# iacopo97/Multimodal-SAM-Adapter

Hardware: AMD Instinct MI355X
Metric: images/sec encoder fwd @1024x1024 RGB+LiDAR ViT-L (higher is better)
Workload: dtype split-operand MFMA: fp16 hi + e5m2 cross terms (h8c / h8 planes, ViT / interaction / up-conv GEMMs) fp16 hi/lo pairs x3 (TwinConvNeXt: f3 planes) and bf16 hi/lo x3 (neck, head); attention blocks with the rel-pos terms fused: every contraction on one fp16 MFMA (q, k, v, P rounded to fp16) in the bloc

## Files before the change

include/mmsa.h:

```cpp
#ifndef MMSA_H
#define MMSA_H
#include <stddef.h>
#include <stdint.h>
#ifdef __cplusplus
extern "C" {
#endif

#ifdef MMSA_BUILDING_LIBRARY
typedef hipStream_t mmsa_stream_t;
#else
typedef void* mmsa_stream_t;
#endif

#include "mmsa_version.h"
int mmsa_version(void);
const char* mmsa_last_error(void);

int mmsa_debug_poison_lds(unsigned pattern, mmsa_stream_t stream);
int mmsa_event_create(void** ev);
int mmsa_event_record(void* ev, mmsa_stream_t stream);
int mmsa_event_elapsed_ms(void* start, void* stop, float* ms);
int mmsa_event_destroy(void* ev);

enum { MMSA_ACT_NONE = 0, MMSA_ACT_GELU = 1, MMSA_ACT_RELU = 2, MMSA_ACT_RELU6 = 3, MMSA_ACT_HSWISH = 4, MMSA_ACT_SIGMOID = 5 };

enum { MMSA_DT_F32 = 0, MMSA_DT_F16 = 1, MMSA_DT_F64 = 2 };

enum { MMSA_FMT_B3 = 0, MMSA_FMT_H8 = 1, MMSA_FMT_H8C = 2, MMSA_FMT_F3 = 3, MMSA_FMT_W8 = 4  };

int mmsa_ms_deform_attn_forward(const void* value, const int64_t* spatial_shapes, const int64_t* level_start_index,
                                const void* sampling_loc, const void* attn_weight, void* out, int batch,
                                int spatial_size, int num_heads, int channels, int num_levels, int num_query,
                                int num_point, int im2col_step, int dtype, mmsa_stream_t stream);

int mmsa_ms_deform_attn_backward(const void* value, const int64_t* spatial_shapes, const int64_t* level_start_index,
                                 const void* sampling_loc, const void* attn_weight, const void* grad_output,
                                 void* grad_value, void* grad_sampling_loc, void* grad_attn_weight, int batch,
                                 int spatial_size, int num_heads, int channels, int num_levels, int num_query,
                                 int num_point, int im2col_step, int dtype, mmsa_stream_t stream);

int mmsa_msda_fused(const float* value, const int64_t* spatial_shapes, const int64_t* level_start_index,
                    const float* raw, long ldraw, const float* ref_points, float* out, long ldo,
                    uint16_t* out_planes, long ldop , int out_fmt , int batch,
                    int spatial_size, int num_heads, int channels, int num_levels, int num_query, int num_point,
                    float* clamp_max , mmsa_stream_t stream);

int mmsa_msda_fused_planes(const uint16_t* value_planes, long ldvp, int lo_bytes, const int64_t* spatial_shapes, const int64_t* level_start_index,
                           const float* raw, long ldraw, const float* ref_points, float* out, long ldo,
                           uint16_t* out_planes, long ldop, int out_fmt, int batch,
                           int spatial_size, int num_heads, int channels, int num_levels, int num_query, int num_point,
                           float* clamp_max, mmsa_stream_t stream);

int mmsa_rowstats_finalize(const float* rowstats, int rows, int strips, int D, float eps, float* mean_rstd, mmsa_stream_t stream);

int mmsa_zero_bytes(void* p, size_t bytes, mmsa_stream_t stream);
int mmsa_gemm_split3(const float* A, const uint16_t* Ap, long lda, long strideA,
                     const uint16_t* Wp, long strideW,
                     const float* bias, long strideBias, const float* colscale, const float* resid, long ldr,
                     long strideR, int resid_mod, float beta, float* C, long ldc, long strideC,
                     uint16_t* Cp, long ldcp, long strideCp, int M, int N, int K,
                     int batch, int act, float alpha, int out_mode, int ps_H, int ps_W, int ps_C, int fmt, int cp_fmt,
                     int max_grid, float* rowstats_out, const float* rownorm_mean_rstd, const float* rownorm_colsum, int flavour,
                     float* clamp_max , mmsa_stream_t stream);

int mmsa_convnext_mlp_fused(const uint16_t* Ap, long lda, long strideA, const uint16_t* W1p, long strideW1, const uint16_t* W2p,
                            long strideW2, const float* b1, const float* b2, const float* gamma, float* x, long ldx, long strideX,
                            int M, int C, int batch, int max_grid, int fmt,
                            float* clamp_max , mmsa_stream_t stream);

int mmsa_split_planes(const float* src, long ld, int rows, int cols, int cols_pad, uint16_t* planes, int kind,
                      float* clamp_max , mmsa_stream_t stream);

int mmsa_attention(const float* qkv, long ldq, const float* qkv_bias, const float* rp, float* out, long ldo, int B,
                   int H, int W, int heads, int head_dim, int window_size, float scale, mmsa_stream_t stream);
int mmsa_attention_planes(const uint16_t* qkv_planes, long ldq, const uint16_t* bias_planes, const float* rp,
                          uint16_t* out_planes, long ldo, int B, int H, int W, int heads, int head_dim,
                          int window_size, float scale, int out_fmt ,
                          int v_fmt ,
                          float* max_abs_logit , mmsa_stream_t stream);

int mmsa_relpos_bias(const float* qkv, long ldq, const float* Rh, const float* Rw, float* rp, int B, int H, int W,
                     int heads, int head_dim, int window_size, mmsa_stream_t stream);
int mmsa_relpos_bias_planes(const uint16_t* qkv_planes, long ldq, const float* Rh, const float* Rw,
                            float* rp, int B, int H, int W, int heads, int head_dim, int window_size, mmsa_stream_t stream);

int mmsa_layernorm_rows(const float* x, long ldx, const float* w, const float* b, float eps, float* y, long ldy,
                        float* y2, long ldy2, uint16_t* y_planes, long ldp ,
                        int rows, int C, int map_mode, int map_H, int map_W, int group_rows, long w_gstride, long y_gcol,
                        int y_wrap, int plane_fmt , float* clamp_max ,
                        mmsa_stream_t stream);

int mmsa_colstats(const float* x, long ldx, long strideB, const float* wrow, int B, int HW, int C, double* out,
                  int out_is_zero , mmsa_stream_t stream);

int mmsa_ffrm_finalize(const double* stats, int B, int HW, int C, float mean_w, float mean_b, const float* Wc,
                       const float* gn_w, const float* gn_b, float* mean_o, float* rstd_o, float* mult_o,
                       float* scratch , mmsa_stream_t stream);
int mmsa_lnhw_apply(const float* x, long ldx, const float* mean, const float* rstd, const float* mult, const float* w,
                    const float* bias, float* y, long ldy, int B, int HW, int C, mmsa_stream_t stream);

int mmsa_dwconv_nhwc(const float* x, long ldx, long xstrideB, const float* w, const float* bias, float* y, long ldy,
                     long ystrideB, uint16_t* y_planes, long ldp, long pstrideB , int planes_fmt ,
                     int B, int H, int W, int C, int k, int act,
                     int imgs_per_group ,
                     float* rowstats ,
                     float* clamp_max , mmsa_stream_t stream);
int mmsa_gconv_nhwc(const float* x, long ldx, const float* w, const float* bias, float* y, long ldy, int B, int H,
                    int W, int G, int cin_g, int cout_g, int k, int act, mmsa_stream_t stream);
int mmsa_gfe_qkv_conv(const float* x, long ldx, const float* w, float* y, long ldy, int B, int H, int W, int G, int cin_g, int cout_g,
                      int* covered, mmsa_stream_t stream);
int mmsa_dwpair_gate(const float* x, long ldx, const float* w, float* y, long ldy, uint16_t* y_planes, long ldp, int B, int H,
                     int W, int C, mmsa_stream_t stream);
int mmsa_im2col_nchw(const float* x, int B, int Ctot, int c0, int Cin, int H, int W, int p, float* out, int Kpad,
                     mmsa_stream_t stream);

long mmsa_gram_tn_scratch_bytes(int B, int P, int c);
int mmsa_gram_tn(const float* X, long ldx, const float* Y, long ldy, long strideB, double* G , int B, int P, int c,
                 int nblk, void* scratch, long scratch_bytes, mmsa_stream_t stream);
int mmsa_chanattn_build(const double* G, const double* sq, long sq_strideB, const double* sk, long sk_strideB,
                        const float* temp, const float* Wp, uint16_t* planes , int B, int c, int cpad,
                        int heads, mmsa_stream_t stream);
int mmsa_gffm_build(const double* E, uint16_t* x_planes, uint16_t* y_planes , int B, int c,
                    int cpad, mmsa_stream_t stream);
int mmsa_gelu_gate(const float* x, long ldx, float* y, long ldy, long rows, int C, mmsa_stream_t stream);
int mmsa_pool_hw(const float* z, long ldz, float* out, long ldo, int B, int H, int W, int C, mmsa_stream_t stream);
int mmsa_ca_apply(const float* z, long ldz, const float* att, long lda, float* out, long ldo,
                  uint16_t* out_planes, long ldp , int B, int H, int W, int C, mmsa_stream_t stream);

int mmsa_tail_fuse(const float* cmap, long ldc, long cstrideB, const float* xtok, long ldx, const float* bn_scale,
                   const float* bn_shift, float* out, uint16_t* out_planes , long ldp,
                   int B, int Hc, int Wc, int Hx, int Wx, int C, mmsa_stream_t stream);

int mmsa_global_attention_planes(const uint16_t* qkv_planes, long ldq, const uint16_t* bias_planes, const uint16_t* relpos_planes,
                                 uint16_t* out_planes, long ldo, int B, int H, int W, int heads, int head_dim, float scale,
                                 int out_fmt , int v_fmt ,
                                 float* max_abs_logit , mmsa_stream_t stream);

int mmsa_window_attention_planes(const uint16_t* qkv_planes, long ldq, const uint16_t* bias_planes,
                                 const uint16_t* relpos_planes, const uint16_t* selector, uint16_t* out_planes, long ldo, int B, int H, int W,
                                 int heads, int head_dim, int window_size, float scale, int out_fmt ,
                                 int v_fmt , float* max_abs_logit , mmsa_stream_t stream);

int mmsa_nchw_to_planes(const float* src, long strideB, uint16_t* planes, long ldp, int B, int C, long HW,
                        mmsa_stream_t stream);
int mmsa_head_fuse(const float* z0, const float* z1, int H1, int W1, const float* z2, int H2, int W2, const float* z3,
                   int H3, int W3, long ld, const float* bn_scale, const float* bn_shift, uint16_t* planes, long ldp,
                   float* out32, long ldo, int B, int H, int W, int C, int act, mmsa_stream_t stream);
int mmsa_tokens_to_nchw(const float* src, long ld, float* dst, int B, long HW, int C, mmsa_stream_t stream);

int mmsa_bilinear_accum_nchw(const float* src, long src_strideB, int B, int C, int hs, int ws, float* dst, int Hd, int Wd, int y0, int x0,
                             int hc, int wc, float* count, int accumulate, mmsa_stream_t stream);
int mmsa_div_count_nchw(float* x, const float* count, int B, int C, long HW, mmsa_stream_t stream);
int mmsa_argmax_nchw(const float* x, unsigned char* out, int B, int C, long HW, mmsa_stream_t stream);
int mmsa_crop_batch_nchw(const float* src, int B, int C, int H, int W, const int* windows, int n, float* dst, int hc, int wc,
                         mmsa_stream_t stream);
int mmsa_slide_argmax(const float* logits, int n, int C, int hs, int ws, const int* windows, unsigned char* out, int B, int H, int W,
                      int hc, int wc, int* uncovered, mmsa_stream_t stream);
int mmsa_slide_argmax_resized(const float* logits, int n, int C, int hs, int ws, const int* windows, unsigned char* out, int B, int H, int W,
                              int hc, int wc, int Hd, int Wd, int Hcut, int Wcut, int* uncovered, mmsa_stream_t stream);

enum { MMSA_PRE_U8 = 0, MMSA_PRE_F32 = 1 };
int mmsa_preprocess_nhwc(const void* src0, int dtype0, const void* src1, int dtype1, int B, int Hs, int Ws, const float* mean,
                         const float* sinv, const int* div255, const int* swap, const float* pad_val, float* dst, int H, int W,
                         mmsa_stream_t stream);
int mmsa_preprocess_crops(const void* src0, int dtype0, const void* src1, int dtype1, int B, int Hs, int Ws, const float* mean,
                          const float* sinv, const int* div255, const int* swap, const float* pad_val, int H, int W, const int* windows,
                          int n, float* dst, int hc, int wc, mmsa_stream_t stream);
int mmsa_preprocess_resize_nhwc(const void* src0, int dtype0, const void* src1, int dtype1, int B, int Hs, int Ws, const float* mean,
                                const float* sinv, const int* div255, const int* swap, const float* pad_val, float* dst, int H, int W,
                                int Hr, int Wr, const int* xofs, const void* xcoef, const int* yofs, const void* ycoef, int fixed_point,
                                mmsa_stream_t stream);
int mmsa_preprocess_resize_crops(const void* src0, int dtype0, const void* src1, int dtype1, int B, int Hs, int Ws, const float* mean,
                                 const float* sinv, const int* div255, const int* swap, const float* pad_val, int H, int W, const int* windows,
                                 int n, float* dst, int hc, int wc, int Hr, int Wr, const int* xofs, const void* xcoef, const int* yofs,
                                 const void* ycoef, int fixed_point, mmsa_stream_t stream);

int mmsa_eval_confusion_u8(const unsigned char* pred, const unsigned char* label, int B, int H, int W, int Hl, int Wl, const unsigned char* lut,
                           int C, const int* ymap, const int* xmap, const int* slots, int n_slots, int64_t* counts, mmsa_stream_t stream);
int mmsa_slide_argmax_eval(const float* logits, int n, int C, int hs, int ws, const int* windows, unsigned char* out, int B, int H, int W,
                           int hc, int wc, int* uncovered, const unsigned char* label, int Hl, int Wl, const unsigned char* lut, const int* ymap,
                           const int* xmap, const int* slots, int n_slots, int64_t* counts, mmsa_stream_t stream);

int mmsa_render_u8(const unsigned char* pred, long pred_image_stride, long pred_row_stride, int B, int h, int w, const unsigned* palette, int npal,
                   int palette_reverse, const unsigned char* src, int Hs, int Ws, int src_reverse, double opacity, double one_minus_opacity,
                   unsigned char* out, mmsa_stream_t stream);
int mmsa_render_denorm_f32(const unsigned char* pred, long pred_image_stride, long pred_row_stride, int B, int h, int w, const unsigned* palette, int npal,
                           int palette_reverse, const float* src, int Cs, int Hs, int Ws, const float* mean, const float* std, int to_rgb, int mul255,
                           double opacity, double one_minus_opacity, unsigned char* out, mmsa_stream_t stream);

#ifdef __cplusplus
}
#endif
#endif
```

include/mmsa_version.h:

```cpp
#ifndef MMSA_VERSION_H
#define MMSA_VERSION_H
#define MMSA_ABI_VERSION 109
#endif
```

multimodal-sam-adapter_amd/mmsa/head.py:

```python
import torch
import torch.nn as nn

from . import lib
from . import ops
from .params import Node, _attach


class SegformerHead(nn.Module):
    def __init__(self, interpolate_mode="bilinear", in_channels=None, channels=None, *, num_classes=None, dropout_ratio=0.1,
                 conv_cfg=None, norm_cfg=None, act_cfg=dict(type="ReLU"), in_index=-1, input_transform="multiple_select",
                 loss_decode=None, ignore_index=255, sampler=None, align_corners=False, init_cfg=None, **kwargs):
        super().__init__()
        if in_channels is None or channels is None or num_classes is None:
            raise TypeError("SegformerHead: in_channels, channels and num_classes are required")
        if not isinstance(in_channels, (list, tuple)) or not isinstance(in_index, (list, tuple)) or len(in_channels) != len(in_index):
            raise AssertionError("SegformerHead: in_channels and in_index must be lists of equal length")
        if not 1 <= len(in_channels) <= 4:
            raise NotImplementedError("mmsa SegformerHead: 1..4 input maps")
        if interpolate_mode != "bilinear" or align_corners:
            raise NotImplementedError("mmsa SegformerHead: only interpolate_mode='bilinear', align_corners=False (the reference configs)")
        if norm_cfg is None or norm_cfg.get("type") not in ("BN", "SyncBN"):
            raise NotImplementedError("mmsa SegformerHead: norm_cfg must be BN / SyncBN (eval: running-statistics affine)")
        if act_cfg is None or act_cfg.get("type") != "ReLU":
            raise NotImplementedError("mmsa SegformerHead: act_cfg must be ReLU")
        if channels % 8:
            raise NotImplementedError("mmsa SegformerHead: channels must be a multiple of 8")
        self.in_channels, self.in_index, self.channels = list(in_channels), list(in_index), channels
        self.num_classes, self.dropout_ratio, self.align_corners = num_classes, dropout_ratio, align_corners
        self.interpolate_mode, self.ignore_index, self.norm_cfg, self.act_cfg = interpolate_mode, ignore_index, norm_cfg, act_cfg
        n = len(in_channels)
        g = torch.Generator().manual_seed(0)

        def conv_w(co, ci):
            return torch.randn(co, ci, 1, 1, generator=g) * (2.0 / ci) ** 0.5

        def bn(prefix):
            _attach(self, prefix + ".weight", torch.ones(channels))
            _attach(self, prefix + ".bias", torch.zeros(channels))
            _attach(self, prefix + ".running_mean", torch.zeros(channels), buffer=True)
            _attach(self, prefix + ".running_var", torch.ones(channels), buffer=True)
            _attach(self, prefix + ".num_batches_tracked", torch.zeros((), dtype=torch.long), buffer=True)

        _attach(self, "conv_seg.weight", torch.randn(num_classes, channels, 1, 1, generator=g) * 0.01)
        _attach(self, "conv_seg.bias", torch.zeros(num_classes))
        self.add_module("convs", Node())
        for i, ci in enumerate(in_channels):
            _attach(self, f"convs.{i}.conv.weight", conv_w(channels, ci))
            bn(f"convs.{i}.bn")
        _attach(self, "fusion_conv.conv.weight", conv_w(channels, channels * n))
        bn("fusion_conv.bn")
        self._packed = None
        self._bufs = {}
        self.register_load_state_dict_post_hook(lambda m, _: m.invalidate())
        self.eval()

    def invalidate(self):
        self._packed = None

    def train(self, mode=True):
        if mode:
            raise NotImplementedError("mmsa: the MI355X decode head implements the inference forward path only")
        return super().train(False)

    def init_weights(self):
        pass

    def forward_test(self, inputs, img_metas=None, test_cfg=None):
        return self.forward(inputs)

    def forward_train(self, inputs, img_metas, gt_semantic_seg, train_cfg):
        raise NotImplementedError("mmsa: the MI355X decode head implements the inference forward path only (no losses)")

    @torch.no_grad()
    def _pack(self, dev):
        sd = {k: v.detach().to(dev, torch.float32) for k, v in self.state_dict().items() if v.dtype.is_floating_point}
        ch, n = self.channels, len(self.in_channels)

        def bn_affine(p):
            s = sd[p + ".weight"] / torch.sqrt(sd[p + ".running_var"] + 1e-5)
            return s.contiguous(), (sd[p + ".bias"] - sd[p + ".running_mean"] * s).contiguous()

        pk = {"branch": []}
        wf = sd["fusion_conv.conv.weight"].reshape(ch, ch * n)
        for i, ci in enumerate(self.in_channels):
            s, t = bn_affine(f"convs.{i}.bn")
            w = sd[f"convs.{i}.conv.weight"].reshape(ch, ci) * s[:, None]
            pk["branch"].append(dict(w=ops.split_planes(w.contiguous()), shift=t,
                                     wf=ops.split_planes(wf[:, ch * i:ch * (i + 1)].contiguous())))
        pk["fs"], pk["ft"] = bn_affine("fusion_conv.bn")
        ncp = ops.pad32(self.num_classes)
        wc = torch.zeros(ncp, ch, device=dev)
        wc[:self.num_classes] = sd["conv_seg.weight"].reshape(self.num_classes, ch)
        bc = torch.zeros(ncp, device=dev)
        bc[:self.num_classes] = sd["conv_seg.bias"]
        pk["wc"], pk["bc"], pk["ncp"] = ops.split_planes(wc), bc, ncp
        return pk

    def _buf(self, name, shape, dtype=torch.float32, dev=None):
        name = getattr(self, "buf_tag", "") + name
        t = self._bufs.get(name)
        if t is None or tuple(t.shape) != tuple(shape) or t.device != dev:
            t = torch.zeros(shape, dtype=dtype, device=dev)
            self._bufs[name] = t
        return t

    def _planes(self, name, rows, cols, dev):
        kp = ops.pad32(cols)
        return ops.Planes(self._buf(name, (rows, 2 * kp), torch.int16, dev), rows, cols, kp)

    @torch.no_grad()
    def forward(self, inputs, out=None):
        x0 = inputs[self.in_index[0]]
        if not x0.is_cuda:
            raise RuntimeError("mmsa SegformerHead: inputs must live on the GPU (there is no CPU path)")
        with torch.cuda.device(x0.device):
            return self._forward(inputs, out)

    def _forward(self, inputs, out=None):
        xs = [inputs[i] for i in self.in_index]
        x0 = xs[0]
        dev = x0.device
        if self._packed is None or self._packed["wc"].p.device != dev:
            self._packed = self._pack(dev)
        pk = self._packed
        B, _, H, W = x0.shape
        ch = self.channels
        zs = []
        for i, (x, ci) in enumerate(zip(xs, self.in_channels)):
            if x.dtype != torch.float32 or x.dim() != 4 or x.shape[0] != B or x.shape[1] != ci:
                raise RuntimeError(f"mmsa SegformerHead: input {i} must be fp32 [B={B}, {ci}, h, w], got {tuple(x.shape)} {x.dtype}")
            x = x.contiguous()
            h, w = x.shape[2:]
            rows = B * h * w
            xp = getattr(inputs[self.in_index[i]], "_mmsa_planes", None)
            if not isinstance(xp, ops.Planes) or xp.n != rows or xp.k != ci or xp.p.device != dev or not xp.live():
                xp = self._planes(f"x{i}", rows, ci, dev)
                lib.call("mmsa_nchw_to_planes", x.data_ptr(), ci * h * w, xp.p.data_ptr(), 2 * xp.kpad, B, ci, h * w, ops._stream())
            br = pk["branch"][i]
            yp = self._planes(f"y{i}", rows, ch, dev)
            ops.gemm(xp, br["w"], bias=br["shift"], act="relu", out_planes=yp)
            z = self._buf(f"z{i}", (rows, ch), dev=dev)
            ops.gemm(yp, br["wf"], z)
            zs.append((z, h, w))
        fp = self._planes("fused", B * H * W, ch, dev)
        lv = zs[1:] + [(None, 0, 0)] * (4 - len(zs))
        lib.call("mmsa_head_fuse", zs[0][0].data_ptr(),
                 lv[0][0].data_ptr() if lv[0][0] is not None else None, lv[0][1], lv[0][2],
                 lv[1][0].data_ptr() if lv[1][0] is not None else None, lv[1][1], lv[1][2],
                 lv[2][0].data_ptr() if lv[2][0] is not None else None, lv[2][1], lv[2][2],
                 ch, pk["fs"].data_ptr(), pk["ft"].data_ptr(), fp.p.data_ptr(), 2 * fp.kpad, None, 0, B, H, W, ch, ops.ACT["relu"],
                 ops._stream())
        lt = self._buf("logit_tokens", (B * H * W, pk["ncp"]), dev=dev)
        ops.gemm(fp, pk["wc"], lt, bias=pk["bc"])
        if out is None:
            out = torch.empty(B, self.num_classes, H, W, device=dev)
        elif (tuple(out.shape) != (B, self.num_classes, H, W) or out.dtype != torch.float32 or out.device != dev or not out.is_contiguous()):
            raise RuntimeError(f"mmsa SegformerHead: out must be a contiguous fp32 [{B}, {self.num_classes}, {H}, {W}] tensor on {dev}")
        lib.call("mmsa_tokens_to_nchw", lt.data_ptr(), pk["ncp"], out.data_ptr(), B, H * W, self.num_classes, ops._stream())
        return out
```

multimodal-sam-adapter_amd/mmsa/lib.py:

```python
import ctypes
import os
from ctypes import c_char_p, c_double, c_float, c_int, c_long, c_void_p, POINTER

_HERE = os.path.dirname(os.path.abspath(__file__))
LIB_PATH = os.environ.get("MMSA_LIB") or os.path.join(_HERE, "libmmsa_hip.so")

if not os.path.exists(LIB_PATH):
    raise RuntimeError(
        f"{LIB_PATH} not found: the MI355X HIP library is required (no CPU/PyTorch fallback exists). "
        "Build it with: python multimodal-sam-adapter_amd/build.py")

import torch

_lib = ctypes.CDLL(LIB_PATH)

P = c_void_p
I = c_int
L = c_long
F = c_float

SIGNATURES = {
    "mmsa_version": [],
    "mmsa_last_error": [],
    "mmsa_debug_poison_lds": [ctypes.c_uint, P],
    "mmsa_event_create": [POINTER(c_void_p)],
    "mmsa_event_record": [P, P],
    "mmsa_event_elapsed_ms": [P, P, POINTER(c_float)],
    "mmsa_event_destroy": [P],
    "mmsa_ms_deform_attn_forward": [P, P, P, P, P, P, I, I, I, I, I, I, I, I, I, P],
    "mmsa_ms_deform_attn_backward": [P, P, P, P, P, P, P, P, P, I, I, I, I, I, I, I, I, I, P],
    "mmsa_msda_fused": [P, P, P, P, L, P, P, L, P, L, I, I, I, I, I, I, I, I, P, P],
    "mmsa_msda_fused_planes": [P, L, I, P, P, P, L, P, P, L, P, L, I, I, I, I, I, I, I, I, P, P],
    "mmsa_gemm_split3": [P, P, L, L, P, L, P, L, P, P, L, L, I, F, P, L, L, P, L, L, I, I, I, I, I, F, I, I, I, I, I, I, I, P, P, P, I, P, P],
    "mmsa_convnext_mlp_fused": [P, L, L, P, L, P, L, P, P, P, P, L, L, I, I, I, I, I, P, P],
    "mmsa_rowstats_finalize": [P, I, I, I, F, P, P],
    "mmsa_zero_bytes": [P, ctypes.c_size_t, P],
    "mmsa_split_planes": [P, L, I, I, I, P, I, P, P],
    "mmsa_attention": [P, L, P, P, P, L, I, I, I, I, I, I, F, P],
    "mmsa_attention_planes": [P, L, P, P, P, L, I, I, I, I, I, I, F, I, I, P, P],
    "mmsa_relpos_bias": [P, L, P, P, P, I, I, I, I, I, I, P],
    "mmsa_relpos_bias_planes": [P, L, P, P, P, I, I, I, I, I, I, P],
    "mmsa_layernorm_rows": [P, L, P, P, F, P, L, P, L, P, L, I, I, I, I, I, I, L, L, I, I, P, P],
    "mmsa_colstats": [P, L, L, P, I, I, I, P, I, P],
    "mmsa_ffrm_finalize": [P, I, I, I, F, F, P, P, P, P, P, P, P, P],
    "mmsa_lnhw_apply": [P, L, P, P, P, P, P, P, L, I, I, I, P],
    "mmsa_dwconv_nhwc": [P, L, L, P, P, P, L, L, P, L, L, I, I, I, I, I, I, I, I, P, P, P],
    "mmsa_dwpair_gate": [P, L, P, P, L, P, L, I, I, I, I, P],
    "mmsa_gconv_nhwc": [P, L, P, P, P, L, I, I, I, I, I, I, I, I, P],
    "mmsa_gfe_qkv_conv": [P, L, P, P, L, I, I, I, I, I, I, POINTER(c_int), P],
    "mmsa_im2col_nchw": [P, I, I, I, I, I, I, I, P, I, P],
    "mmsa_gram_tn": [P, L, P, L, L, P, I, I, I, I, P, L, P],
    "mmsa_gram_tn_scratch_bytes": [I, I, I],
    "mmsa_chanattn_build": [P, P, L, P, L, P, P, P, I, I, I, I, P],
    "mmsa_gffm_build": [P, P, P, I, I, I, P],
    "mmsa_gelu_gate": [P, L, P, L, L, I, P],
    "mmsa_pool_hw": [P, L, P, L, I, I, I, I, P],
    "mmsa_ca_apply": [P, L, P, L, P, L, P, L, I, I, I, I, P],
    "mmsa_tail_fuse": [P, L, L, P, L, P, P, P, P, L, I, I, I, I, I, I, P],
    "mmsa_global_attention_planes": [P, L, P, P, P, L, I, I, I, I, I, F, I, I, P, P],
    "mmsa_window_attention_planes": [P, L, P, P, P, P, L, I, I, I, I, I, I, F, I, I, P, P],
    "mmsa_nchw_to_planes": [P, L, P, L, I, I, L, P],
    "mmsa_head_fuse": [P, P, I, I, P, I, I, P, I, I, L, P, P, P, L, P, L, I, I, I, I, I, P],
    "mmsa_tokens_to_nchw": [P, L, P, I, L, I, P],
    "mmsa_bilinear_accum_nchw": [P, L, I, I, I, I, P, I, I, I, I, I, I, P, I, P],
    "mmsa_div_count_nchw": [P, P, I, I, L, P],
    "mmsa_argmax_nchw": [P, P, I, I, L, P],
    "mmsa_crop_batch_nchw": [P, I, I, I, I, P, I, P, I, I, P],
    "mmsa_slide_argmax": [P, I, I, I, I, P, P, I, I, I, I, I, P, P],
    "mmsa_slide_argmax_resized": [P, I, I, I, I, P, P, I, I, I, I, I, I, I, I, I, P, P],
    "mmsa_preprocess_nhwc": [P, I, P, I, I, I, I, P, P, P, P, P, P, I, I, P],
    "mmsa_preprocess_crops": [P, I, P, I, I, I, I, P, P, P, P, P, I, I, P, I, P, I, I, P],
    "mmsa_preprocess_resize_nhwc": [P, I, P, I, I, I, I, P, P, P, P, P, P, I, I, I, I, P, P, P, P, I, P],
    "mmsa_preprocess_resize_crops": [P, I, P, I, I, I, I, P, P, P, P, P, I, I, P, I, P, I, I, I, I, P, P, P, P, I, P],
    "mmsa_eval_confusion_u8": [P, P, I, I, I, I, I, P, I, P, P, P, I, P, P],
    "mmsa_slide_argmax_eval": [P, I, I, I, I, P, P, I, I, I, I, I, P, P, I, I, P, P, P, P, I, P, P],
    "mmsa_render_u8": [P, L, L, I, I, I, P, I, I, P, I, I, I, c_double, c_double, P, P],
    "mmsa_render_denorm_f32": [P, L, L, I, I, I, P, I, I, P, I, I, I, P, P, I, I, c_double, c_double, P, P],
}
_RESTYPES = {"mmsa_last_error": c_char_p, "mmsa_gram_tn_scratch_bytes": c_long}

for _name, _args in SIGNATURES.items():
    _fn = getattr(_lib, _name)
    _fn.argtypes = _args
    _fn.restype = _RESTYPES.get(_name, c_int)


ABI_VERSION = 109
if _lib.mmsa_version() != ABI_VERSION:
    raise RuntimeError(f"{LIB_PATH}: ABI version {_lib.mmsa_version()} but mmsa/lib.py binds version {ABI_VERSION} (include/mmsa.h MMSA_ABI_VERSION): "
                       "rebuild with python multimodal-sam-adapter_amd/build.py")


def last_error() -> str:
    return _lib.mmsa_last_error().decode()


POISON_LDS = os.environ.get("MMSA_DEBUG_POISON_LDS") == "1"


def call(name, *args):
    if POISON_LDS and not name.startswith(("mmsa_event", "mmsa_debug")) and args:
        _lib.mmsa_debug_poison_lds(0x7FC07FC0, args[-1])
    rc = getattr(_lib, name)(*args)
    if rc != 0:
        raise RuntimeError(f"{name} failed (rc={rc}): {last_error()}")


def version() -> int:
    return _lib.mmsa_version()


raw = _lib
```

Before: 64.84.

## Fuse SegFormer head upsample-merge, BN/ReLU and classifier into one kernel

Adds a head_fuse_cls kernel that bilinearly upsamples and sums the level features, applies the BN affine and ReLU, then runs the 1x1 classifier with fp32 MFMA and writes NCHW logits directly. Low-res level patches are staged in LDS per tile and channel chunks are double-buffered. This removes the fused-planes intermediate, the separate classifier GEMM and the tokens-to-NCHW transpose pass. In exchange the classifier runs in fp32 MFMA instead of the split bf16 planes GEMM, which is slower per flop, and the path only applies when there are at most 32 classes.

```diff
diff --git a/include/mmsa.h b/include/mmsa.h
--- a/include/mmsa.h
+++ b/include/mmsa.h
@@ -147,6 +147,9 @@
                    int H3, int W3, long ld, const float* bn_scale, const float* bn_shift, uint16_t* planes, long ldp,
                    float* out32, long ldo, int B, int H, int W, int C, int act, mmsa_stream_t stream);
 int mmsa_tokens_to_nchw(const float* src, long ld, float* dst, int B, long HW, int C, mmsa_stream_t stream);
+int mmsa_head_fuse_cls(const float* z0, const float* z1, int H1, int W1, const float* z2, int H2, int W2, const float* z3,
+                       int H3, int W3, long ld, const float* bn_scale, const float* bn_shift, const float* wc, const float* bias,
+                       int num_classes, float* logits, long img_stride, int B, int H, int W, int C, int act, mmsa_stream_t stream);
 
 int mmsa_bilinear_accum_nchw(const float* src, long src_strideB, int B, int C, int hs, int ws, float* dst, int Hd, int Wd, int y0, int x0,
                              int hc, int wc, float* count, int accumulate, mmsa_stream_t stream);
diff --git a/include/mmsa_version.h b/include/mmsa_version.h
--- a/include/mmsa_version.h
+++ b/include/mmsa_version.h
@@ -1,4 +1,4 @@
 #ifndef MMSA_VERSION_H
 #define MMSA_VERSION_H
-#define MMSA_ABI_VERSION 109
+#define MMSA_ABI_VERSION 110
 #endif
diff --git a/multimodal-sam-adapter_amd/csrc/head_cls.hip b/multimodal-sam-adapter_amd/csrc/head_cls.hip
--- /dev/null
+++ b/multimodal-sam-adapter_amd/csrc/head_cls.hip
@@ -0,0 +1,254 @@
+#include "common.h"
+
+#define HC_POOL 128
+#define HC_WLD 36
+#define HC_TH 8
+#define HC_TW 16
+
+struct HeadClsLevels {
+  const float* z[3];
+  int H[3], W[3];
+  float rh[3], rw[3];
+  int pbase[3], pitch[3], ph[3];
+  int stmask, used;
+};
+
+__host__ __device__ __forceinline__ void hc_src(int d, float r, int n, int& i0, int& i1, float& l) {
+  float s = fmaf((float)d + 0.5f, r, -0.5f);
+  s = s < 0.f ? 0.f : s;
+  const int i = (int)s;
+  i0 = i < n - 1 ? i : n - 1;
+  i1 = i0 + (i0 < n - 1 ? 1 : 0);
+  l = s - (float)i0;
+}
+
+template <int NLV, bool ALLST>
+__global__ __launch_bounds__(512, ALLST ? 4 : 2) void head_fuse_cls_kernel(const float* __restrict__ z0, long ld, HeadClsLevels lv,
+                                                               const float* __restrict__ bn_scale, const float* __restrict__ bn_shift,
+                                                               const float* __restrict__ wc, const float* __restrict__ bias, int num_classes,
+                                                               float* __restrict__ logits, long img_stride, int H, int W, int C, int tilesX,
+                                                               int relu, int vec) {
+  __shared__ float4 patch[2][HC_POOL * 8];
+  __shared__ float wsl[2][32 * HC_WLD];
+  __shared__ float4 bnl[2][16];
+  constexpr int NL = NLV > 0 ? NLV : 1;
+  const int b = blockIdx.z;
+  const int tx0 = (blockIdx.x % tilesX) * HC_TW, ty0 = (blockIdx.x / tilesX) * HC_TH;
+  const int t = threadIdx.x, lane = t & 63, wave = t >> 6, l15 = lane & 15, kk = lane >> 4;
+  const int hlast = min(ty0 + HC_TH - 1, H - 1), wlast = min(tx0 + HC_TW - 1, W - 1);
+  auto is_staged = [&](const int i) { return ALLST || ((lv.stmask >> i) & 1) != 0; };
+
+  const int wq = min(tx0 + l15, wlast), hq = min(ty0 + wave, hlast);
+  int oh[NL], ow[NL];
+  int p00[NL], p10[NL], dw[NL];
+  float lh[NL], lw[NL];
+#pragma unroll
+  for (int i = 0; i < NLV; ++i) {
+    int a1, h0, h1, w0, w1;
+    float l_;
+    hc_src(ty0, lv.rh[i], lv.H[i], oh[i], a1, l_);
+    hc_src(tx0, lv.rw[i], lv.W[i], ow[i], a1, l_);
+    hc_src(wq, lv.rw[i], lv.W[i], w0, w1, lw[i]);
+    hc_src(hq, lv.rh[i], lv.H[i], h0, h1, lh[i]);
+    dw[i] = w1 - w0;
+    if (is_staged(i)) {
+      p00[i] = lv.pbase[i] + (h0 - oh[i]) * lv.pitch[i] + (w0 - ow[i]);
+      p10[i] = lv.pbase[i] + (h1 - oh[i]) * lv.pitch[i] + (w0 - ow[i]);
+    } else {
+      p00[i] = h0 * lv.W[i] + w0;
+      p10[i] = h1 * lv.W[i] + w0;
+    }
+  }
+
+  const float* z0p = z0 + (((long)b * H + hq) * W + wq) * ld + 4 * kk;
+  const int nit = (lv.used * 8 + 511) >> 9;
+  const float* sp[2];
+  unsigned svalid = 0;
+#pragma unroll
+  for (int it = 0; it < 2; ++it) {
+    const int gp = (t + 512 * it) >> 3, q = t & 7;
+    const float* src = z0p;
+#pragma unroll
+    for (int i = 0; i < NLV; ++i) {
+      const int np = lv.pitch[i] * lv.ph[i];
+      const bool in = is_staged(i) && gp >= lv.pbase[i] && gp < lv.pbase[i] + np;
+      const int local = in ? gp - lv.pbase[i] : 0;
+      const int py = local / lv.pitch[i], px = local - py * lv.pitch[i];
+      const int sy = min(oh[i] + py, lv.H[i] - 1), sx = min(ow[i] + px, lv.W[i] - 1);
+      const float* cand = lv.z[i] + (((long)b * lv.H[i] + sy) * lv.W[i] + sx) * ld + 4 * q;
+      src = in ? cand : src;
+      svalid |= in ? 1u << it : 0u;
+    }
+    sp[it] = src;
+  }
+  const float* wcp = t < 256 ? wc + (long)(t >> 3) * C + 4 * (t & 7) : (t < 264 ? bn_scale : bn_shift) + 4 * (t & 7);
+
+  f32x4 acc[2];
+#pragma unroll
+  for (int nt = 0; nt < 2; ++nt) {
+    const float bv = bias[nt * 16 + l15];
+    acc[nt] = (f32x4){bv, bv, bv, bv};
+  }
+
+  float4 zr[2], pr[2], wr;
+  auto load_chunk = [&](const int c0) {
+#pragma unroll
+    for (int jj = 0; jj < 2; ++jj) zr[jj] = *reinterpret_cast<const float4*>(z0p + c0 + 16 * jj);
+#pragma unroll
+    for (int it = 0; it < 2; ++it)
+      if (it < nit) pr[it] = *reinterpret_cast<const float4*>(sp[it] + c0);
+    wr = *reinterpret_cast<const float4*>(wcp + c0);
+  };
+  auto store_chunk = [&](const int buf) {
+#pragma unroll
+    for (int it = 0; it < 2; ++it) {
+      const int gp = (t + 512 * it) >> 3, q = t & 7;
+      if (svalid & (1u << it)) patch[buf][gp * 8 + (q ^ ((gp >> 1) & 3))] = pr[it];
+    }
+    if (t < 256) *reinterpret_cast<float4*>(&wsl[buf][(t >> 3) * HC_WLD + 4 * (t & 7)]) = wr;
+    else if (t < 272) bnl[buf][t - 256] = wr;
+  };
+#pragma unroll
+  for (int it = 0; it < 2; ++it) pr[it] = make_float4(0.f, 0.f, 0.f, 0.f);
+  load_chunk(0);
+  store_chunk(0);
+  __syncthreads();
+
+  for (int c0 = 0; c0 < C; c0 += 32) {
+    const int buf = (c0 >> 5) & 1;
+    float v[8] = {zr[0].x, zr[0].y, zr[0].z, zr[0].w, zr[1].x, zr[1].y, zr[1].z, zr[1].w};
+    const bool more = c0 + 32 < C;
+    if (more) load_chunk(c0 + 32);
+
+#pragma unroll
+    for (int i = 0; i < NLV; ++i) {
+      const int pq[4] = {p00[i], p00[i] + dw[i], p10[i], p10[i] + dw[i]};
+      const float w00 = (1.f - lh[i]) * (1.f - lw[i]), w01 = (1.f - lh[i]) * lw[i], w10 = lh[i] * (1.f - lw[i]), w11 = lh[i] * lw[i];
+#pragma unroll
+      for (int jj = 0; jj < 2; ++jj) {
+        float4 tp[4];
+        if (is_staged(i)) {
+#pragma unroll
+          for (int k = 0; k < 4; ++k) tp[k] = patch[buf][pq[k] * 8 + ((4 * jj + kk) ^ ((pq[k] >> 1) & 3))];
+        } else {
+          const float* zi = lv.z[i] + (long)b * lv.H[i] * lv.W[i] * ld + c0 + 4 * kk + 16 * jj;
+#pragma unroll
+          for (int k = 0; k < 4; ++k) tp[k] = *reinterpret_cast<const float4*>(zi + (long)pq[k] * ld);
+        }
+        const float4 t00 = tp[0], t01 = tp[1], t10 = tp[2], t11 = tp[3];
+        v[4 * jj + 0] += w00 * t00.x + w01 * t01.x + w10 * t10.x + w11 * t11.x;
+        v[4 * jj + 1] += w00 * t00.y + w01 * t01.y + w10 * t10.y + w11 * t11.y;
+        v[4 * jj + 2] += w00 * t00.z + w01 * t01.z + w10 * t10.z + w11 * t11.z;
+        v[4 * jj + 3] += w00 * t00.w + w01 * t01.w + w10 * t10.w + w11 * t11.w;
+      }
+    }
+#pragma unroll
+    for (int jj = 0; jj < 2; ++jj) {
+      const float4 s4 = bnl[buf][4 * jj + kk], f4 = bnl[buf][8 + 4 * jj + kk];
+      const float s[4] = {s4.x, s4.y, s4.z, s4.w}, f[4] = {f4.x, f4.y, f4.z, f4.w};
+      float4 bq[2];
+#pragma unroll
+      for (int nt = 0; nt < 2; ++nt) bq[nt] = *reinterpret_cast<const float4*>(&wsl[buf][(nt * 16 + l15) * HC_WLD + 16 * jj + 4 * kk]);
+#pragma unroll
+      for (int e = 0; e < 4; ++e) {
+        const float y = v[4 * jj + e] * s[e] + f[e];
+        const float a = relu ? fmaxf(y, 0.f) : y;
+#pragma unroll
+        for (int nt = 0; nt < 2; ++nt) {
+          const float bf = e == 0 ? bq[nt].x : e == 1 ? bq[nt].y : e == 2 ? bq[nt].z : bq[nt].w;
+          acc[nt] = __builtin_amdgcn_mfma_f32_16x16x4f32(a, bf, acc[nt], 0, 0, 0);
+        }
+      }
+    }
+    if (more) store_chunk(buf ^ 1);
+    __syncthreads();
+  }
+
+  const int oy = ty0 + wave, ox = tx0 + 4 * kk;
+  if (oy >= H || ox >= W) return;
+#pragma unroll
+  for (int nt = 0; nt < 2; ++nt) {
+    const int cls = nt * 16 + l15;
+    if (cls >= num_classes) continue;
+    float* dst = logits + (long)b * img_stride + ((long)cls * H + oy) * W + ox;
+    if (vec) {
+      *reinterpret_cast<float4*>(dst) = make_float4(acc[nt][0], acc[nt][1], acc[nt][2], acc[nt][3]);
+    } else {
+#pragma unroll
+      for (int r = 0; r < 4; ++r)
+        if (ox + r < W) dst[r] = acc[nt][r];
+    }
+  }
+}
+
+template <int NLV>
+static void launch_head_fuse_cls(dim3 grid, hipStream_t stream, const float* z0, long ld, const HeadClsLevels& lv, const float* bn_scale,
+                                 const float* bn_shift, const float* wc, const float* bias, int num_classes, float* logits, long img_stride, int H,
+                                 int W, int C, int tilesX, int relu, int vec) {
+  if (lv.stmask == (1 << NLV) - 1)
+    hipLaunchKernelGGL((head_fuse_cls_kernel<NLV, true>), grid, dim3(512), 0, stream, z0, ld, lv, bn_scale, bn_shift, wc, bias, num_classes, logits,
+                       img_stride, H, W, C, tilesX, relu, vec);
+  else
+    hipLaunchKernelGGL((head_fuse_cls_kernel<NLV, false>), grid, dim3(512), 0, stream, z0, ld, lv, bn_scale, bn_shift, wc, bias, num_classes, logits,
+                       img_stride, H, W, C, tilesX, relu, vec);
+}
+
+extern "C" int mmsa_head_fuse_cls(const float* z0, const float* z1, int H1, int W1, const float* z2, int H2, int W2, const float* z3, int H3, int W3,
+                                  long ld, const float* bn_scale, const float* bn_shift, const float* wc, const float* bias, int num_classes,
+                                  float* logits, long img_stride, int B, int H, int W, int C, int act, hipStream_t stream) {
+  MMSA_CHECK_ARG(z0 && bn_scale && bn_shift && wc && bias && logits, "head_fuse_cls: null pointer");
+  MMSA_CHECK_ARG(B > 0 && B <= 65535 && H > 0 && W > 0 && C > 0 && C % 32 == 0, "head_fuse_cls: bad shape (C=%d must be a multiple of 32, B=%d at most 65535)", C, B);
+  MMSA_CHECK_ARG(num_classes > 0 && num_classes <= 32, "head_fuse_cls: %d classes (1..32 supported)", num_classes);
+  MMSA_CHECK_ARG(act == ACT_NONE || act == ACT_RELU, "head_fuse_cls: activation %d (none or ReLU)", act);
+  MMSA_CHECK_ARG(ld >= C && ld % 4 == 0, "head_fuse_cls: row stride %ld", ld);
+  MMSA_CHECK_ARG(((((uintptr_t)bn_scale) | ((uintptr_t)bn_shift) | ((uintptr_t)z0) | ((uintptr_t)wc)) & 15) == 0,
+                 "head_fuse_cls: z0 / bn_scale / bn_shift / wc must be 16-byte aligned");
+  MMSA_CHECK_ARG((long)H * W < (1L << 27), "head_fuse_cls: too many pixels for the 32-bit index arithmetic");
+  MMSA_CHECK_ARG(img_stride >= (long)num_classes * H * W, "head_fuse_cls: image stride %ld < num_classes*H*W", img_stride);
+  const int tx = cdiv(W, HC_TW), ty = cdiv(H, HC_TH);
+  HeadClsLevels lv;
+  int n = 0;
+  const float* zs[3] = {z1, z2, z3};
+  const int hs[3] = {H1, H2, H3}, wsz[3] = {W1, W2, W3};
+  for (int i = 0; i < 3; ++i) {
+    lv.z[i] = nullptr; lv.H[i] = lv.W[i] = 1; lv.rh[i] = lv.rw[i] = 1.f; lv.pbase[i] = 0; lv.pitch[i] = 1; lv.ph[i] = 0;
+  }
+  lv.stmask = 0; lv.used = 0;
+  for (int i = 0; i < 3; ++i) {
+    if (!zs[i]) continue;
+    MMSA_CHECK_ARG(hs[i] > 0 && wsz[i] > 0 && (long)hs[i] * wsz[i] < (1L << 27), "head_fuse_cls: level %d has bad size", i + 1);
+    MMSA_CHECK_ARG((((uintptr_t)zs[i]) & 15) == 0, "head_fuse_cls: level %d must be 16-byte aligned", i + 1);
+    lv.z[n] = zs[i]; lv.H[n] = hs[i]; lv.W[n] = wsz[i];
+    lv.rh[n] = (float)hs[i] / (float)H;
+    lv.rw[n] = (float)wsz[i] / (float)W;
+    int PH = 1, PW = 1, i0, i1, j0, j1;
+    float l_;
+    for (int r = 0; r < ty; ++r) {
+      hc_src(r * HC_TH, lv.rh[n], hs[i], i0, i1, l_);
+      hc_src(H - 1 < r * HC_TH + HC_TH - 1 ? H - 1 : r * HC_TH + HC_TH - 1, lv.rh[n], hs[i], j0, j1, l_);
+      if (j1 - i0 + 1 > PH) PH = j1 - i0 + 1;
+    }
+    for (int c = 0; c < tx; ++c) {
+      hc_src(c * HC_TW, lv.rw[n], wsz[i], i0, i1, l_);
+      hc_src(W - 1 < c * HC_TW + HC_TW - 1 ? W - 1 : c * HC_TW + HC_TW - 1, lv.rw[n], wsz[i], j0, j1, l_);
+      if (j1 - i0 + 1 > PW) PW = j1 - i0 + 1;
+    }
+    if (PH <= HC_POOL && PW <= HC_POOL && PH * PW <= HC_POOL - lv.used) {
+      lv.stmask |= 1 << n;
+      lv.pbase[n] = lv.used; lv.pitch[n] = PW; lv.ph[n] = PH;
+      lv.used += PH * PW;
+    }
+    ++n;
+  }
+  const dim3 grid(tx * ty, 1, B);
+  const int vec = W % 4 == 0 && img_stride % 4 == 0 && (((uintptr_t)logits) & 15) == 0;
+  const int relu = act == ACT_RELU ? 1 : 0;
+  switch (n) {
+    case 0: launch_head_fuse_cls<0>(grid, stream, z0, ld, lv, bn_scale, bn_shift, wc, bias, num_classes, logits, img_stride, H, W, C, tx, relu, vec); break;
+    case 1: launch_head_fuse_cls<1>(grid, stream, z0, ld, lv, bn_scale, bn_shift, wc, bias, num_classes, logits, img_stride, H, W, C, tx, relu, vec); break;
+    case 2: launch_head_fuse_cls<2>(grid, stream, z0, ld, lv, bn_scale, bn_shift, wc, bias, num_classes, logits, img_stride, H, W, C, tx, relu, vec); break;
+    default: launch_head_fuse_cls<3>(grid, stream, z0, ld, lv, bn_scale, bn_shift, wc, bias, num_classes, logits, img_stride, H, W, C, tx, relu, vec); break;
+  }
+  MMSA_CHECK_LAUNCH("head_fuse_cls");
+  return MMSA_OK;
+}
diff --git a/multimodal-sam-adapter_amd/mmsa/head.py b/multimodal-sam-adapter_amd/mmsa/head.py
--- a/multimodal-sam-adapter_amd/mmsa/head.py
+++ b/multimodal-sam-adapter_amd/mmsa/head.py
@@ -7,6 +7,8 @@
 
 
 class SegformerHead(nn.Module):
+    fuse_cls = True
+
     def __init__(self, interpolate_mode="bilinear", in_channels=None, channels=None, *, num_classes=None, dropout_ratio=0.1,
                  conv_cfg=None, norm_cfg=None, act_cfg=dict(type="ReLU"), in_index=-1, input_transform="multiple_select",
                  loss_decode=None, ignore_index=255, sampler=None, align_corners=False, init_cfg=None, **kwargs):
@@ -88,13 +90,22 @@
             pk["branch"].append(dict(w=ops.split_planes(w.contiguous()), shift=t,
                                      wf=ops.split_planes(wf[:, ch * i:ch * (i + 1)].contiguous())))
         pk["fs"], pk["ft"] = bn_affine("fusion_conv.bn")
-        ncp = ops.pad32(self.num_classes)
+        wc, bc = self._pack_classifier(dev)
+        pk["wc"], pk["wc32"], pk["bc"], pk["ncp"] = ops.split_planes(wc), wc, bc, wc.shape[0]
+        return pk
+
+    @torch.no_grad()
+    def _pack_classifier(self, dev):
+        ch, ncp = self.channels, ops.pad32(self.num_classes)
+        sd = self.state_dict()
         wc = torch.zeros(ncp, ch, device=dev)
-        wc[:self.num_classes] = sd["conv_seg.weight"].reshape(self.num_classes, ch)
+        wc[:self.num_classes] = sd["conv_seg.weight"].detach().to(dev, torch.float32).reshape(self.num_classes, ch)
         bc = torch.zeros(ncp, device=dev)
-        bc[:self.num_classes] = sd["conv_seg.bias"]
-        pk["wc"], pk["bc"], pk["ncp"] = ops.split_planes(wc), bc, ncp
-        return pk
+        bc[:self.num_classes] = sd["conv_seg.bias"].detach().to(dev, torch.float32)
+        return wc.contiguous(), bc
+
+    def _fuses_cls(self):
+        return bool(self.fuse_cls) and self.channels % 32 == 0 and self.num_classes <= 32
 
     def _buf(self, name, shape, dtype=torch.float32, dev=None):
         name = getattr(self, "buf_tag", "") + name
@@ -142,19 +153,23 @@
             z = self._buf(f"z{i}", (rows, ch), dev=dev)
             ops.gemm(yp, br["wf"], z)
             zs.append((z, h, w))
+        if out is None:
+            out = torch.empty(B, self.num_classes, H, W, device=dev)
+        elif (tuple(out.shape) != (B, self.num_classes, H, W) or out.dtype != torch.float32 or out.device != dev or not out.is_contiguous()):
+            raise RuntimeError(f"mmsa SegformerHead: out must be a contiguous fp32 [{B}, {self.num_classes}, {H}, {W}] tensor on {dev}")
+        lv = zs[1:] + [(None, 0, 0)] * (4 - len(zs))
+        levels = (lv[0][0].data_ptr() if lv[0][0] is not None else None, lv[0][1], lv[0][2],
+                  lv[1][0].data_ptr() if lv[1][0] is not None else None, lv[1][1], lv[1][2],
+                  lv[2][0].data_ptr() if lv[2][0] is not None else None, lv[2][1], lv[2][2])
+        if self._fuses_cls():
+            lib.call("mmsa_head_fuse_cls", zs[0][0].data_ptr(), *levels, ch, pk["fs"].data_ptr(), pk["ft"].data_ptr(), pk["wc32"].data_ptr(),
+                     pk["bc"].data_ptr(), self.num_classes, out.data_ptr(), self.num_classes * H * W, B, H, W, ch, ops.ACT["relu"], ops._stream())
+            return out
         fp = self._planes("fused", B * H * W, ch, dev)
-        lv = zs[1:] + [(None, 0, 0)] * (4 - len(zs))
-        lib.call("mmsa_head_fuse", zs[0][0].data_ptr(),
-                 lv[0][0].data_ptr() if lv[0][0] is not None else None, lv[0][1], lv[0][2],
-                 lv[1][0].data_ptr() if lv[1][0] is not None else None, lv[1][1], lv[1][2],
-                 lv[2][0].data_ptr() if lv[2][0] is not None else None, lv[2][1], lv[2][2],
+        lib.call("mmsa_head_fuse", zs[0][0].data_ptr(), *levels,
                  ch, pk["fs"].data_ptr(), pk["ft"].data_ptr(), fp.p.data_ptr(), 2 * fp.kpad, None, 0, B, H, W, ch, ops.ACT["relu"],
                  ops._stream())
         lt = self._buf("logit_tokens", (B * H * W, pk["ncp"]), dev=dev)
         ops.gemm(fp, pk["wc"], lt, bias=pk["bc"])
-        if out is None:
-            out = torch.empty(B, self.num_classes, H, W, device=dev)
-        elif (tuple(out.shape) != (B, self.num_classes, H, W) or out.dtype != torch.float32 or out.device != dev or not out.is_contiguous()):
-            raise RuntimeError(f"mmsa SegformerHead: out must be a contiguous fp32 [{B}, {self.num_classes}, {H}, {W}] tensor on {dev}")
         lib.call("mmsa_tokens_to_nchw", lt.data_ptr(), pk["ncp"], out.data_ptr(), B, H * W, self.num_classes, ops._stream())
         return out
diff --git a/multimodal-sam-adapter_amd/mmsa/lib.py b/multimodal-sam-adapter_amd/mmsa/lib.py
--- a/multimodal-sam-adapter_amd/mmsa/lib.py
+++ b/multimodal-sam-adapter_amd/mmsa/lib.py
@@ -62,6 +62,7 @@
     "mmsa_nchw_to_planes": [P, L, P, L, I, I, L, P],
     "mmsa_head_fuse": [P, P, I, I, P, I, I, P, I, I, L, P, P, P, L, P, L, I, I, I, I, I, P],
     "mmsa_tokens_to_nchw": [P, L, P, I, L, I, P],
+    "mmsa_head_fuse_cls": [P, P, I, I, P, I, I, P, I, I, L, P, P, P, P, I, P, L, I, I, I, I, I, P],
     "mmsa_bilinear_accum_nchw": [P, L, I, I, I, I, P, I, I, I, I, I, I, P, I, P],
     "mmsa_div_count_nchw": [P, P, I, I, L, P],
     "mmsa_argmax_nchw": [P, P, I, I, L, P],
@@ -85,7 +86,7 @@
     _fn.restype = _RESTYPES.get(_name, c_int)
 
 
-ABI_VERSION = 109
+ABI_VERSION = 110
 if _lib.mmsa_version() != ABI_VERSION:
     raise RuntimeError(f"{LIB_PATH}: ABI version {_lib.mmsa_version()} but mmsa/lib.py binds version {ABI_VERSION} (include/mmsa.h MMSA_ABI_VERSION): "
                        "rebuild with python multimodal-sam-adapter_amd/build.py")
```

Result: no change. 65.48, median of 6 (+1.0%).
